# YuyaW-0118/Sparse-Matrix-Linear-Equations

Hardware: AMD Instinct MI355X
Metric: fp64 SpMV GFLOP/s + achieved HBM GB/s vs roofline; CG iters/sec (higher is better)
Workload: dtype f64; 1 GPU; merge-path CSR SpMV fp64, 1 RHS, batch of 4 pwtk-shaped matrices per step per GPU (configs[1]); m=217918, nnz=11524432, batch=4, parallelism=independent SpMV batches, 1 GPU(s)

## Files before the change

include/mspmv.h:

```cpp
#ifndef MSPMV_H
#define MSPMV_H

#include <stddef.h>

#ifndef MSPMV_API
#define MSPMV_API __attribute__((visibility("default")))
#endif

#ifdef __cplusplus
extern "C" {
#endif

typedef enum mspmv_status {
    MSPMV_OK = 0,
    MSPMV_ERR_INVALID = 1,
    MSPMV_ERR_HIP = 2,
    MSPMV_ERR_OOM = 3,
    MSPMV_ERR_BREAKDOWN = 4,
    MSPMV_ERR_RCCL = 5,
    MSPMV_ERR_UNSUPPORTED = 6,
    MSPMV_ERR_IO = 7,
    MSPMV_ERR_STALL = 8,
    MSPMV_ERR_FAULT = 9
} mspmv_status;
// ... 92 lines not shown
MSPMV_API mspmv_status mspmv_color_greedy(const mspmv_csr_d *a, int *colors, int *num_colors);
MSPMV_API mspmv_status mspmv_csr_permute_sym(const mspmv_csr_d *a, const int *perm, int *ro, int *ci, double *va);
MSPMV_API mspmv_status mspmv_ilu0_create_colored(const mspmv_csr_d *a, const int *colors, int device,
                                                 mspmv_ilu0 *out);
MSPMV_API mspmv_status mspmv_ilu0_colors(mspmv_ilu0 m, int *num_colors, int *perm);
MSPMV_API mspmv_status mspmv_ilu0_apply_dev(mspmv_handle a, mspmv_ilu0 m, const double *d_B, double *d_X, int L);
MSPMV_API mspmv_status mspmv_dpbicgstab_ilu0_multi(mspmv_handle a, mspmv_ilu0 m, const double *B, double *X, int L,
                                                   int max_iters, double tolerance, int *iters,
                                                   double *max_err_hist, int hist_cap);
MSPMV_API mspmv_status mspmv_dpbicgstab_ilu0_multi_dev(mspmv_handle a, mspmv_ilu0 m, const double *d_B, double *d_X,
                                                       int L, int max_iters, double tolerance, int *iters,
                                                       double *max_err_hist, int hist_cap);

MSPMV_API mspmv_status mspmv_ic0_create_colored(const mspmv_csr_d *a, const int *colors, int device, double *shift,
                                                mspmv_ic0 *out);
MSPMV_API mspmv_status mspmv_ic0_colors(mspmv_ic0 m, int *num_colors, int *perm);
MSPMV_API mspmv_status mspmv_ic0_apply_dev(mspmv_handle a, mspmv_ic0 m, const double *d_B, double *d_X, int L);

MSPMV_API mspmv_status mspmv_time_spmm_dev(mspmv_handle h, const double *d_X, double *d_Y, int L, int reps,
                                 size_t flush_bytes, double *avg_ms);
MSPMV_API mspmv_status mspmv_time_spmm_batch_dev(int count, const mspmv_handle *hs, const double *const *d_X,
                                                 double *const *d_Y, int L, int reps, double *step_ms,
                                                 double *tile_kernel_ms, int *kernels_per_step);
MSPMV_API mspmv_status mspmv_time_stream_read(int device, size_t bytes, int reps, double *gbps);
MSPMV_API mspmv_status mspmv_last_kernel_ms(mspmv_handle h, double *tile_kernel_ms, int *kernels_per_call);

MSPMV_API mspmv_status mspmv_tile_plan(mspmv_handle h, int L, int *num_tiles, int *tile_items, int *num_carries,
                                       mspmv_coord *bounds);
MSPMV_API mspmv_status mspmv_tile_streams(mspmv_handle h, int *tiles_cols16, int *tiles_dict);
MSPMV_API mspmv_status mspmv_plan_dict_tiles(mspmv_handle h, int L, int *tiles_dict);
MSPMV_API mspmv_status mspmv_plan_block_tiles(mspmv_handle h, int L, int *tiles_blk);
MSPMV_API mspmv_status mspmv_plan_block_rounds(mspmv_handle h, int L, int *tiles_two_rounds);
MSPMV_API mspmv_status mspmv_plan_block_records(mspmv_handle h, int L, int *chunks_compact, int *chunks_escaped);
enum mspmv_slab_stat {
    MSPMV_SLAB_STAT_BLOCKS = 0,
    MSPMV_SLAB_STAT_GROUPS,
    MSPMV_SLAB_STAT_UNITS,
    MSPMV_SLAB_STAT_UNITS_MAX,
    MSPMV_SLAB_STAT_ROWS_MAX,
    MSPMV_SLAB_STAT_EMPTY_BLOCKS,
    MSPMV_SLAB_STAT_CARRIES,
    MSPMV_SLAB_STAT_CHUNKS_FULL,
    MSPMV_SLAB_STAT_CHUNKS_ENTRY_CUT,
    MSPMV_SLAB_STAT_RUNS_CUT,
    MSPMV_SLAB_STAT_CHUNKS_LONG,
    MSPMV_SLAB_STAT_LONG_RUNS_MAX,
    MSPMV_SLAB_STAT_LG0,
    MSPMV_SLAB_STAT_SEGMENTS = MSPMV_SLAB_STAT_LG0 + 7,
    MSPMV_SLAB_STAT_SEGMENTS_MAX,
    MSPMV_SLAB_STAT_SEGMENTS_FULL,
    MSPMV_SLAB_STAT_SEGMENTS_RAGGED,
    MSPMV_SLAB_STAT_PACK_8X1,
    MSPMV_SLAB_STAT_PACK_4X2,
    MSPMV_SLAB_STAT_PACK_2X3,
    MSPMV_SLAB_STAT_PACK_2X4,
    MSPMV_SLAB_STAT_PACK_1X5,
    MSPMV_SLAB_STAT_UNPACKED_1 = MSPMV_SLAB_STAT_PACK_1X5 + 4,
    MSPMV_SLAB_STAT_MEDIUM_2 = MSPMV_SLAB_STAT_UNPACKED_1 + 8,
    MSPMV_SLAB_STAT_SLICES_ODD = MSPMV_SLAB_STAT_MEDIUM_2 + 7,
    MSPMV_SLAB_STAT_SLICES_PARTIAL,
    MSPMV_SLAB_STAT_LONG_1,
    MSPMV_SLAB_STAT_LONG_2,
    MSPMV_SLAB_STAT_LONG_3PLUS,
    MSPMV_SLAB_STAT_PIECES_MAX,
    MSPMV_SLAB_STAT_SEGS_PIECES_ONLY,
    MSPMV_SLAB_STAT_SEGS_REFILL,
// ... 36 lines not shown
```

sparse-matrix-linear-equations_amd/csrc/mspmv_api.hip:

```cpp
#include "mspmv_internal.h"

#include <algorithm>
#include <atomic>
#include <chrono>
#include <cstdio>
#include <cstring>
#include <map>
#include <mutex>
#include <vector>

namespace mspmv {

static thread_local std::string g_err;

void set_error(const std::string &msg) { g_err = msg; }

hipError_t launch_flush(void *p, size_t bytes, hipStream_t s, bool fresh);

}

unsigned long long mspmv_next_generation()
{
    static std::atomic<unsigned long long> next{1};
    return next.fetch_add(1, std::memory_order_relaxed);
// ... 933 lines not shown
    const TilePlan *plan = nullptr;
    ST_TRY(product_plan(h, L, &plan));
    *tiles_blk = plan->d_blk ? plan->num_tiles_blk : 0;
    return MSPMV_OK;
}

mspmv_status mspmv_plan_block_rounds(mspmv_handle h, int L, int *tiles_two_rounds)
{
    ST_TRY(check_handle(h));
    if (!tiles_two_rounds)
        return invalid("null out pointer");
    if (!supported_L(L))
        return (set_error("L must be one of 1, 2, 4, 8, 16"), MSPMV_ERR_UNSUPPORTED);
    const TilePlan *plan = nullptr;
    ST_TRY(product_plan(h, L, &plan));
    *tiles_two_rounds = plan->d_blk ? plan->blk_two_rounds : 0;
    return MSPMV_OK;
}

mspmv_status mspmv_plan_block_records(mspmv_handle h, int L, int *chunks_compact, int *chunks_escaped)
{
    ST_TRY(check_handle(h));
    if (!chunks_compact || !chunks_escaped)
        return invalid("null out pointer");
    if (!supported_L(L))
        return (set_error("L must be one of 1, 2, 4, 8, 16"), MSPMV_ERR_UNSUPPORTED);
    const TilePlan *plan = nullptr;
    ST_TRY(product_plan(h, L, &plan));
    *chunks_compact = plan->d_recs ? plan->blk_rec_compact : 0;
    *chunks_escaped = plan->d_recs ? plan->blk_rec_escaped : 0;
    return MSPMV_OK;
}

mspmv_status mspmv_slab_plan_stats(mspmv_handle h, int L, long long *stats, int count, int *on_slab)
{
    ST_TRY(check_handle(h));
    if (!on_slab || (count > 0 && !stats))
        return invalid("null out pointer");
    if (!supported_L(L))
        return (set_error("L must be one of 1, 2, 4, 8, 16"), MSPMV_ERR_UNSUPPORTED);
    const TilePlan *plan = nullptr;
    ST_TRY(product_plan(h, L, &plan));
    *on_slab = plan->slab ? 1 : 0;
    if (!plan->slab)
        return MSPMV_OK;
    SlabStats s = plan->slab->stats;
    s.v[MSPMV_SLAB_STAT_BLOCKS] = plan->num_tiles;
    s.v[MSPMV_SLAB_STAT_GROUPS] = plan->slab->groups;
    s.v[MSPMV_SLAB_STAT_CARRIES] = plan->num_carries;
    for (int i = 0; i < count && i < MSPMV_SLAB_STAT_COUNT; ++i)
        stats[i] = s.v[i];
    return MSPMV_OK;
}

mspmv_status mspmv_block_record_encode(const unsigned short *offsets, int wc, unsigned *entries, int *escaped)
{
    if (!entries || !escaped || (wc > 0 && !offsets))
        return invalid("null pointer");
    if (wc < 0 || wc > 64)
        return invalid("a chunk holds 0..64 pattern columns");
    *escaped = blk_rec_encode(offsets, wc, entries) ? 0 : 1;
    return MSPMV_OK;
}

mspmv_status mspmv_block_record_decode(const unsigned *record, int q, unsigned *offset)
{
// ... 63 lines not shown
```

sparse-matrix-linear-equations_amd/csrc/mspmv_internal.h:

```cpp
#pragma once

#include <hip/hip_runtime.h>

#include <cstdint>
#include <map>
#include <string>
#include <type_traits>
#include <utility>
#include <vector>

#include "mspmv.h"
#include "mspmv_host.h"

static inline hipError_t memset_sync(void *p, int value, size_t bytes)
{
    const hipError_t e = hipMemset(p, value, bytes);
    return e == hipSuccess ? hipStreamSynchronize(nullptr) : e;
}

namespace mspmv {

constexpr int kBlock = 256;
constexpr unsigned kFaultTicket = 1u;
constexpr int kNnzPad = 16;
// ... 96 lines not shown
    double *d_rem_val = nullptr;
};

struct TilePlan {
    int lanes = kBlock;
    int tile_items = 0;
    int snap = 0;
    int num_tiles = 0;
    int2 *d_bounds = nullptr;
    unsigned char *d_split = nullptr;
    unsigned char *d_modes[5] = {nullptr, nullptr, nullptr, nullptr, nullptr};
    int num_carries = 0;
    double *d_carry_val = nullptr;
    int4 *d_fix = nullptr;
    unsigned *d_fix_cnt = nullptr;
    int carry_L = 0;
    int *d_colbase = nullptr;
    unsigned short *d_cols16 = nullptr;
    int num_tiles16 = 0;
    int *d_dict = nullptr;
    int *d_ndict = nullptr;
    unsigned short *d_idx16 = nullptr;
    int num_tiles_dict = 0;
    uint4 *d_blk = nullptr;
    int blk_stride = 0;
    unsigned short *d_pcols = nullptr;
    unsigned *d_recs = nullptr;
    int blk_rec_compact = 0;
    int blk_rec_escaped = 0;
    int num_tiles_blk = 0;
    int num_tiles_reg = 0;
    int blk_rows_max = 8;
    bool blk_spmv = false;
    int blk_two_rounds = 0;
    std::vector<unsigned char> h_blk_reg;
    SlabData *slab = nullptr;
    DiaData *dia = nullptr;
};

struct CgScalars {
    double rs_old;
    double b_norm;
    double alpha;
    double beta;
    double pAp;
    double rs_new;
    double rs_par[2];
    double omega;
    double rho;
};

struct CgControl {
    int iter;
    int done;
    int iters_out;
    int breakdown;
    int iter_par[2];
    int x_pending;
    unsigned fault;
    unsigned fault_no_stop;
};


struct ResidentCg {
    bool ok = false;
    int G = 0, rpt = 0, nzr = 0;
// ... 463 lines not shown
```

sparse-matrix-linear-equations_amd/csrc/mspmv_kernels.hip:

```cpp
#include "mspmv_internal.h"
#include "mspmv_device.h"

#include <algorithm>
#include <type_traits>
#include <cmath>
#include <cstdio>
#include <cstdlib>

namespace mspmv {


template <typename... KArgs, typename... Args>
static void ggl(void (*kernel)(KArgs...), dim3 grid, dim3 block, hipStream_t s, Args... args)
{
    hipLaunchKernelGGL(kernel, grid, block, 0, s, args...);
}

template <bool NT, typename T>
__device__ __forceinline__ T ld_stream(const T *p)
{
    if (NT)
        return __builtin_nontemporal_load(p);
    return *p;
}
// ... 396 lines not shown
    double *head_pub;
    double *y0;
    int num_tiles;
    CgScalars *scal;
    CgControl *ctrl;
    const unsigned char *conv;
    double *partials;
    unsigned *gtickets;
    double *dot_out;
    int m;
    const double *part_in;
    int n_part_in;
    int parity;
    double tol;
    double *hist;
    int hist_cap;
    const int *colbase;
    const unsigned short *cols16;
    const uint4 *blk;
    int blk_stride;
    int all_reg;
    const unsigned short *pcols;
    const unsigned *recs;
    const int *dict;
    const int *ndict;
    const unsigned short *idx16;
    int ld;
    int early_re;
    int blk_rows_max;
    unsigned long long *stamps;
    int tb;
    int blk_spmv;
    int n;
};

enum : int { kModeSpmv = 0, kModeCg = 1, kModeDot = 2 };

__device__ __forceinline__ double2 cg_rp(const TileArgs &a, long long i)
{
    return reinterpret_cast<const double2 *>(a.x)[i];
}
__device__ __forceinline__ void cg_pstore(const TileArgs &a, long long i, double p) { a.p_new[2 * i + 1] = p; }

__device__ __forceinline__ int pslot(int k) { return k ^ ((k >> 3) & 7); }

template <int TB>
__device__ __forceinline__ void tile_sync()
{
    if (TB == 64) {
        __builtin_amdgcn_fence(__ATOMIC_RELEASE, "wavefront");
        __builtin_amdgcn_wave_barrier();
        __builtin_amdgcn_fence(__ATOMIC_ACQUIRE, "wavefront");
    } else {
        __syncthreads();
    }
}

template <int NJ, bool CG>
struct StageRegs {
    int c[NJ];
    double v[NJ];
    double xv[NJ];
    double pv[CG ? NJ : 1];
};
template <int NJ, bool CG, bool NT, int TB = kBlock>
__device__ __forceinline__ void stage_issue(const TileArgs &a, int n0, int nnzt, int colbase, StageRegs<NJ, CG> &st)
// ... 224 lines not shown
                if (CG)
                    x = x + beta * st.pv[s];
                int start = 0;
#pragma unroll
                for (int i = 0; i < kBlkRows; ++i) {
                    const int len = blk_len(d, i);
                    if (i < h && j < len)
                        s_prod[pslot(vofs + start + j)] = st.v[s][i] * x;
                    start += i < h ? len : 0;
                }
            }
        }
    }
}

__device__ __forceinline__ double rows8_sum(const double (&p)[kBlkRows])
{
    const int lane = threadIdx.x & 63;
    const bool b5 = lane & 32, b4 = lane & 16, b3 = lane & 8;
    double q4[4], q2[2];
#pragma unroll
    for (int k = 0; k < 4; ++k)
        q4[k] = (b5 ? p[k + 4] : p[k]) + __shfl_xor(b5 ? p[k] : p[k + 4], 32);
#pragma unroll
    for (int k = 0; k < 2; ++k)
        q2[k] = (b4 ? q4[k + 2] : q4[k]) + __shfl_xor(b4 ? q4[k] : q4[k + 2], 16);
    double v = (b3 ? q2[1] : q2[0]) + __shfl_xor(b3 ? q2[0] : q2[1], 8);
    v += __shfl_xor(v, 4);
    v += __shfl_xor(v, 2);
    v += __shfl_xor(v, 1);
    return v;
}

__device__ __forceinline__ double rows8_sum32(const double (&p)[kBlkRows])
{
    const int lane = threadIdx.x & 63;
    const bool b4 = lane & 16, b3 = lane & 8, b2 = lane & 4;
    double q4[4], q2[2];
#pragma unroll
    for (int k = 0; k < 4; ++k)
        q4[k] = (b4 ? p[k + 4] : p[k]) + __shfl_xor(b4 ? p[k] : p[k + 4], 16);
#pragma unroll
    for (int k = 0; k < 2; ++k)
        q2[k] = (b3 ? q4[k + 2] : q4[k]) + __shfl_xor(b3 ? q4[k] : q4[k + 2], 8);
    double v = (b2 ? q2[1] : q2[0]) + __shfl_xor(b2 ? q2[0] : q2[1], 4);
    v += __shfl_xor(v, 2);
    v += __shfl_xor(v, 1);
    return v;
}

template <bool NT>
__device__ __forceinline__ unsigned blk_pair_rec(const TileArgs &a, int t, int round)
{
    const int lane = threadIdx.x & 63;
    const int slot = 8 * round + 2 * (int)(threadIdx.x >> 6) + (lane >> 5);
    return ld_stream<NT>(a.recs + ((size_t)t * a.blk_stride + slot) * kRecDwords + (lane & 15));
}

template <bool NT, int KR>
__device__ __forceinline__ void blk_rows_pair(const TileArgs &a, int t, unsigned rec, int nd, int r0, int n0,
                                              int colbase)
{
    constexpr int NW = kBlock / 64;
    const int lane = threadIdx.x & 63;
    const int half = lane >> 5, hl = lane & 31;
    const int wave = __builtin_amdgcn_readfirstlane((int)(threadIdx.x >> 6));
    for (int round = 0; round * 2 * NW < nd; ++round) {
        if (round > 0)
            rec = blk_pair_rec<NT>(a, t, round);
        const int di = wave + NW * (2 * round + half);
        const bool valid = di < nd;
        auto dword = [&](int k) { return (unsigned)__shfl((int)rec, (lane & 32) + k); };
        const uint4 d = make_uint4(dword(0), dword(1), dword(2), dword(3));
        const int vofs = d.x & 0xffff, wc = d.x >> 24;
        const int h = d.y & 15, rofs = d.y >> 16;
        double2 v[KR];
        bool in0[KR], in1[KR];
        int start = 0;
#pragma unroll
        for (int i = 0; i < KR; ++i) {
            const int len = blk_len(d, i);
            in0[i] = valid && i < h && 2 * hl < len;
            in1[i] = valid && i < h && 2 * hl + 1 < len;
            v[i] = make_double2(0.0, 0.0);
            if (in0[i])
                v[i] = ld_stream<NT>(reinterpret_cast<const double2 *>(a.vals + n0 + vofs + start + 2 * hl));
            start += i < h ? len : 0;
        }
        const int q = max(min(2 * hl, wc - 1), 0);
        int e;
        const unsigned E = blk_rec_find([&](int i) { return dword(4 + i); }, q, e);
        const unsigned En = dword(4 + min(e + 1, kRecEntries - 1));
        int c0 = colbase + (int)((E & 0xffffu) + (unsigned)q - (E >> 24));
        int c1 = c0 + 1;
        if (2 * hl + 1 < wc && 2 * hl + 1 == (int)((E >> 24) + ((E >> 16) & 255u)))
            c1 = colbase + (int)(En & 0xffffu);
        if (d.y & kRecEscape) {
            const int p = (d.y >> 4) & 7;
            int pstart = 0;
#pragma unroll
            for (int i = 0; i < KR - 1; ++i)
                pstart += i < p ? blk_len(d, i) : 0;
            unsigned cc = 0u;
            if (2 * hl < wc)
                cc = ld_stream<NT>(reinterpret_cast<const unsigned *>(a.cols16 + n0 + vofs + pstart + 2 * hl));
            c0 = colbase + (int)(cc & 0xffffu);
            c1 = 2 * hl + 1 < wc ? colbase + (int)(cc >> 16) : c0 + 1;
        }
        const int base = min(c0, a.n - 2);
        const double2 xx = *reinterpret_cast<const double2 *>(a.x + base);
        const double x0 = base == c0 ? xx.x : xx.y;
        double x1 = xx.y;
        if (c1 != c0 + 1)
            x1 = a.x[c1];
        double pr[kBlkRows];
#pragma unroll
        for (int i = 0; i < kBlkRows; ++i)
            pr[i] = i < KR ? (in0[i] ? v[i].x * x0 : 0.0) + (in1[i] ? v[i].y * x1 : 0.0) : 0.0;
        const double sum = rows8_sum32(pr);
        const int myrow = hl >> 2;
        if (valid && (hl & 3) == 0 && myrow < h)
            a.y[r0 + rofs + myrow] = sum;
    }
}

template <int MODE, bool NT, int TB, typename Head>
__device__ __forceinline__ void blk_rows(const TileArgs &a, int t, const uint4 &bd, int nd, int r0, int n0,
                                         int colbase, double &beta, double &dot, Head &&head)
{
    constexpr bool CG = MODE == kModeCg;
    constexpr int NW = TB / 64;
    const int lane = threadIdx.x & 63;
    const int wave = __builtin_amdgcn_readfirstlane((int)(threadIdx.x >> 6));
    const int myrow = lane >> 3;
    for (int round = 0; round * 2 * NW < nd; ++round) {
        BlkRegs<CG> st;
        double2 ro[2];
#pragma unroll
        for (int s = 0; s < 2; ++s) {
            const int di = wave + NW * (2 * round + s);
            st.c[s] = 0;
            ro[s] = make_double2(0.0, 0.0);
#pragma unroll
            for (int i = 0; i < kBlkRows; ++i)
                st.v[s][i] = 0.0;
            if (di < nd) {
                const uint4 d = blk_read(bd, di);
                const int vofs = d.x & 0xffff, wc = d.x >> 24;
                const int h = d.y & 15, rofs = d.y >> 16;
                int start = 0;
#pragma unroll
                for (int i = 0; i < kBlkRows; ++i) {
                    const int len = blk_len(d, i);
                    if (i < h && lane < len)
// ... 486 lines not shown
        return;
    const int mean = (nnzt + nseg - 1) / nseg;
    int lg = 0;
    while (lg < 6 && (4 << lg) < mean)
        ++lg;
    const int G = 1 << lg;
    const int lane = threadIdx.x & (G - 1);
    auto col = [&](int k) {
        return colbase >= 0 ? colbase + (int)ld_stream<NT>(a.cols16 + n0 + k) : ld_stream<NT>(a.cols + n0 + k);
    };
    for (int r = (int)threadIdx.x >> lg; r < nseg; r += kBlock >> lg) {
        const int s0 = r == 0 ? 0 : a.row_offsets[r0 + r] - n0;
        const int e = r < nrows ? a.row_offsets[r0 + r + 1] - n0 : nnzt;
        double v = 0.0;
        for (int k = s0 + lane; k < e; k += G)
            v += ld_stream<NT>(a.vals + n0 + k) * a.x[col(k)];
        for (int off = G >> 1; off > 0; off >>= 1)
            v += __shfl_xor(v, off);
        if (lane == 0) {
            if (r < nrows)
                *(r == 0 ? a.y0 : &a.y[r0 + r]) = v;
            else
                store_sc1(&a.carry_val[t], v);
        }
    }
}

struct BlkSmem {
    double red[kBlock / 64];
    double cval[kBlock];
    int last;
};

template <int MODE, bool NT, int KR = kBlkRows, bool FB = false>
__global__ __launch_bounds__(kBlock) void k_spmv_blk(TileArgs a)
{
    constexpr bool CG = MODE == kModeCg;
    __shared__ BlkSmem sm;
    const int tid = threadIdx.x;
    const int stopped = (MODE != kModeSpmv || a.ctrl) ? a.ctrl->done : 0;
    const int t = xcd_tile(blockIdx.x, a.num_tiles);
    const int2 b0 = a.bounds[t];
    const int colbase = a.colbase[t];
    const uint4 bd =
        (tid & 63) < a.blk_stride ? a.blk[(size_t)t * a.blk_stride + (tid & 63)] : make_uint4(0u, 0u, 0u, 0u);
    const int nblk = (int)(((unsigned)__builtin_amdgcn_readfirstlane((int)bd.y) >> 8) & 255u);
    double beta = 0.0, dot = 0.0;
    bool go = true;
    PartRegs<CG ? kUpdateMaxBlocks / kBlock : 1> pin;
    if constexpr (CG)
        part_load(a.part_in, a.n_part_in, pin);
    if constexpr (MODE == kModeSpmv && KR <= 6) {
        const unsigned rec = blk_pair_rec<NT>(a, t, 0);
        asm volatile("" ::"s"(b0.x), "s"(b0.y), "s"(colbase), "v"(rec));
        if (stopped)
            return;
        const int nrec = (int)(((unsigned)__builtin_amdgcn_readlane((int)rec, 1) >> 8) & 255u);
        if constexpr (FB) {
            if (nrec == 0) {
                const int4 fx = load_fix(a, t);
                a.y0 = fx.z > 0 ? a.head_val + t : a.y + b0.x;
                tile_rows_reg<NT>(a, t, b0.x, b0.y, a.cols16 ? colbase : -1);
                close_split_rows<kBlock>(a, t, fx, 1, 1);
                return;
            }
        }
        blk_rows_pair<NT, KR>(a, t, rec, nrec, b0.x, b0.y, colbase);
        return;
    }
    blk_rows<MODE, NT, kBlock>(a, t, bd, nblk, b0.x, b0.y, colbase, beta, dot, [&]() {
        if (stopped)
            go = false;
        else if constexpr (CG)
// ... 786 lines not shown
    return hipGetLastError();
}

static TileArgs make_args(mspmv_handle_s *h, const TilePlan &plan, const double *X, double *Y, int L)
{
    TileArgs a{};
    a.row_offsets = h->d_row_offsets;
    a.m = h->m;
    a.cols = h->d_cols;
    a.vals = h->d_vals;
    a.x = X;
    a.xr = X;
    a.y = Y;
    a.bounds = plan.d_bounds;
    a.split = plan.d_split;
    a.rmode = plan.d_modes[l_index(L)];
    a.carry_val = plan.d_carry_val;
    a.fix = plan.num_carries ? plan.d_fix : nullptr;
    a.fix_cnt = plan.d_fix_cnt;
    a.fault = h->d_fault;
    a.head_val = plan.d_carry_val + (size_t)std::max(plan.num_tiles, 1) * plan.carry_L;
    a.head_pub = a.head_val + (size_t)std::max(plan.num_tiles, 1) * plan.carry_L;
    a.num_tiles = plan.num_tiles;
    if (L == 1 || plan.d_blk) {
        a.colbase = plan.d_colbase;
        a.cols16 = plan.d_cols16;
        a.blk = plan.d_blk;
        a.blk_stride = plan.blk_stride;
        a.pcols = plan.d_pcols;
        a.recs = plan.d_recs;
        a.all_reg = plan.d_blk && plan.num_tiles_reg == plan.num_tiles && (L == 1 || spmm_blk_enabled());
        a.blk_spmv = L == 1 && plan.blk_spmv;
        a.blk_rows_max = plan.blk_rows_max;
    }
    a.dict = plan.d_dict;
    a.ndict = plan.d_ndict;
    a.idx16 = plan.d_idx16;
    a.ld = L;
    a.early_re = L == 1 ? 1 : 0;
    a.tb = L == 1 ? plan.lanes : kBlock;
    a.n = h->n;
    return a;
}

template <int LL, int I, int MODE>
static void launch_spmm_nt(const TileArgs &a, hipStream_t s, bool nt)
{
    if constexpr (MODE != kModeCg) {
        const dim3 grid(a.num_tiles), block(kBlock);
        dispatch_bool(nt, [&](auto ntc) {
            constexpr bool NT = decltype(ntc)::value;
            if constexpr (spmm_dict_max(LL) > 0) {
                if (a.dict) {
                    ggl(k_spmm_tile<LL, I, MODE, NT, true>, grid, block, s, a);
                    return;
                }
            }
            if (MODE == kModeSpmv && !a.fix)
                ggl(k_spmm_tile<LL, I, MODE, NT, false, false>, grid, block, s, a);
            else
                ggl(k_spmm_tile<LL, I, MODE, NT>, grid, block, s, a);
        });
    }
}

template <int LL, int MODE>
static void launch_spmm_L(const TileArgs &a, hipStream_t s, bool nt)
{
    if constexpr (MODE != kModeCg) {
        if (a.all_reg) {
            const dim3 grid(a.num_tiles), block(kBlock);
            dispatch_bool(nt, [&](auto ntc) {
                constexpr bool NT = decltype(ntc)::value;
                if (a.blk_rows_max <= 6)
                    ggl(k_spmm_blk<LL, MODE, NT, 6>, grid, block, s, a);
                else
                    ggl(k_spmm_blk<LL, MODE, NT>, grid, block, s, a);
            });
            return;
        }
    }
    launch_spmm_nt<LL, (LL >= 16 ? 32 : LL >= 8 ? 24 : 8), MODE>(a, s, nt);
}

template <int MODE>
static void launch_spmv_1(const TileArgs &a, hipStream_t s, bool nt)
{
    const dim3 grid(a.num_tiles), block(kBlock);
    dispatch_bool(nt, [&](auto ntc) {
        constexpr bool NT = decltype(ntc)::value;
        if (MODE == kModeSpmv && a.blk_spmv) {
            if (a.all_reg)
                ggl(k_spmv_blk<kModeSpmv, NT, 6>, grid, block, s, a);
            else
                ggl(k_spmv_blk<kModeSpmv, NT, 6, true>, grid, block, s, a);
        } else if (MODE == kModeDot && a.all_reg) {
            ggl(k_spmv_blk<kModeDot, NT>, grid, block, s, a);
        } else if (MODE == kModeSpmv && a.tb == 64) {
            ggl(k_spmv_tile<kSpmvIpt, kModeSpmv, NT, 64>, grid, dim3(64), s, a);
        } else if (MODE == kModeCg && !a.blk) {
            ggl(k_spmv_tile<kSpmvIpt, MODE, NT, kBlock, false>, grid, block, s, a);
        } else if (MODE == kModeSpmv && !a.fix) {
            ggl(k_spmv_tile<kSpmvIpt, MODE, NT, kBlock, true, false>, grid, block, s, a);
        } else {
            ggl(k_spmv_tile<kSpmvIpt, MODE, NT>, grid, block, s, a);
        }
    });
}

template <int MODE>
static hipError_t launch_tile(const TileArgs &a, int L, hipStream_t s, bool nt)
{
    if (MODE == kModeCg && L != 1)
        return hipErrorInvalidValue;
    return dispatch_L(L, [&](auto Lc) {
        constexpr int LL = decltype(Lc)::value;
        if constexpr (LL == 1)
            launch_spmv_1<MODE>(a, s, nt);
        else
            launch_spmm_L<LL, MODE>(a, s, nt);
        return hipGetLastError();
    });
}

hipError_t launch_spmv_tile_stamped(mspmv_handle_s *h, const TilePlan &plan, const double *d_x, double *d_y,
                                   unsigned long long *d_stamps)
{
    TileArgs a = make_args(h, plan, d_x, d_y, 1);
    if (a.blk_spmv || a.tb == 64 || plan.dia || plan.slab)
        return hipErrorNotSupported;
    a.stamps = d_stamps;
    const dim3 grid(a.num_tiles), block(kBlock);
    if (plan.num_tiles == 0)
        return hipSuccess;
    const bool nt = stream_nt(h);
    dispatch_bool(nt, [&](auto ntc) {
        constexpr bool NT = decltype(ntc)::value;
        if (!a.fix)
            ggl(k_spmv_tile<kSpmvIpt, kModeSpmv, NT, kBlock, true, false, true>, grid, block, h->stream, a);
        else
            ggl(k_spmv_tile<kSpmvIpt, kModeSpmv, NT, kBlock, true, true, true>, grid, block, h->stream, a);
    });
    return hipGetLastError();
}

hipError_t launch_spmm_tile_only(mspmv_handle_s *h, const TilePlan &plan, const double *d_X, double *d_Y, int L,
                                 int ld, CgControl *ctrl)
{
    if (plan.num_tiles == 0)
        return hipSuccess;
    if (plan.dia)
        return launch_dia(h, plan, d_X, d_Y, L, ld, ctrl);
    if (plan.slab) {
        if (plan.slab->L != L || (L == 1 && ctrl))
            return hipErrorInvalidValue;
        return L == 1 ? launch_slab(h, plan, d_X, d_Y) : launch_slab_mm(h, plan, d_X, d_Y, L, ld, ctrl);
// ... 89 lines not shown
```

sparse-matrix-linear-equations_amd/csrc/mspmv_plan.hip:

```cpp
#include "mspmv_internal.h"

#include <algorithm>
#include <cstdlib>
#include <vector>

using namespace mspmv;

void mspmv::free_plan(TilePlan &p)
{
    dev_free(p.d_bounds);
    dev_free(p.d_split);
    for (auto &m : p.d_modes)
        dev_free(m);
    dev_free(p.d_fix);
    dev_free(p.d_fix_cnt);
    dev_free(p.d_carry_val);
    dev_free(p.d_colbase);
    dev_free(p.d_cols16);
    dev_free(p.d_dict);
    dev_free(p.d_ndict);
    dev_free(p.d_idx16);
    dev_free(p.d_blk);
    dev_free(p.d_pcols);
    dev_free(p.d_recs);
// ... 2 lines not shown
    free_dia(p.dia);
    p.dia = nullptr;
}

static mspmv_status build_plan(mspmv_handle_s *h, int L, const TilePlan **out, int lanes = 0,
                               const std::vector<int2> *fixed = nullptr);

static mspmv_status ensure_modes(mspmv_handle_s *h, TilePlan &p, int L)
{
    unsigned char *&m = p.d_modes[l_index(L)];
    if (m)
        return MSPMV_OK;
    mspmv_status st = dev_alloc(&m, (size_t)std::max(p.num_tiles, 1));
    if (st != MSPMV_OK)
        return st;
    hipError_t e = launch_tile_modes(h->d_row_offsets, p.d_bounds, p.d_split, p.num_tiles, L, m, h->stream, p.lanes);
    if (e == hipSuccess)
        e = hipStreamSynchronize(h->stream);
    if (e != hipSuccess) {
        set_error(std::string("tile modes: ") + hipGetErrorString(e));
        dev_free(m);
        m = nullptr;
        return MSPMV_ERR_HIP;
    }
    return MSPMV_OK;
}

static int env_tristate(const char *name)
{
    const char *e = getenv(name);
    return e && *e ? (atoi(e) != 0 ? 1 : 0) : -1;
}

static mspmv_status optional_failed(mspmv_status st, bool forced)
{
    if (forced && st != MSPMV_ERR_UNSUPPORTED)
        return st;
    set_error("");
    (void)hipGetLastError();
    return MSPMV_OK;
}

static mspmv_status keep_optional(mspmv_handle_s *h, int key, TilePlan &p, mspmv_status st, bool forced, int *decision)
{
    if (st != MSPMV_OK) {
        free_plan(p);
        return optional_failed(st, forced);
    }
    h->plans.emplace(key, p);
    *decision = 1;
    return MSPMV_OK;
}

constexpr double kDiaAutoFill = 0.85;
constexpr double kDiaWindowFill = 0.3;

static mspmv_status dia_decide(mspmv_handle_s *h)
{
    h->dia = 0;
    const int sw = env_tristate("MSPMV_DIA");
    if (sw == 0)
        return MSPMV_OK;
    TilePlan p;
    const mspmv_status st = build_dia_plan(h, p, sw == 1 ? 0.0 : kDiaAutoFill, sw == 1 ? 0.0 : kDiaWindowFill);
    return keep_optional(h, kDiaPlanKey, p, st, sw == 1, &h->dia);
}
// ... 189 lines not shown
    if (single && !onewave && p.d_cols16 && spmv_blocks_enabled()) {
        if ((st = dev_alloc(&p.d_blk, (size_t)T * kBlkPerTile)) != MSPMV_OK)
            return fail(st);
        e = launch_build_blocks(h->d_row_offsets, h->d_cols, p.d_bounds, p.d_split, p.d_colbase, T, p.d_blk,
                                h->stream, kBlkPlanChunks);
        std::vector<uint4> hd((size_t)T * kBlkPerTile);
        if (e == hipSuccess)
            e = hipMemcpyAsync(hd.data(), p.d_blk, sizeof(uint4) * hd.size(), hipMemcpyDeviceToHost, h->stream);
        if (e == hipSuccess)
            e = hipStreamSynchronize(h->stream);
        if (e != hipSuccess) {
            set_error(std::string("node blocks: ") + hipGetErrorString(e));
            return fail(MSPMV_ERR_HIP);
        }
        p.h_blk_reg.assign((size_t)T, 0);
        int maxnd = 0, maxh = 0;
        std::vector<unsigned char> reg((size_t)T, 0);
        for (int t = 0; t < T; ++t) {
            const uint4 *d = &hd[(size_t)t * kBlkPerTile];
            const int nd = (int)((d[0].y >> 8) & 255u);
            if (nd == 0)
                continue;
            ++p.num_tiles_blk;
            maxnd = std::max(maxnd, nd);
            for (int i = 0; i < nd; ++i)
                maxh = std::max(maxh, (int)(d[i].y & 15u));
            bool one = true;
            for (int i = 0; i < nd; ++i)
                one = one && ((d[i].x >> 16) & 255u) == 0;
            reg[(size_t)t] = one;
            p.num_tiles_reg += one;
        }
        p.blk_spmv = p.num_tiles_reg > 0 && 2LL * p.num_tiles_reg >= T;
        for (int t = 0; t < T; ++t) {
            const int nd = (int)((hd[(size_t)t * kBlkPerTile].y >> 8) & 255u);
            p.h_blk_reg[(size_t)t] = p.blk_spmv || (reg[(size_t)t] && nd <= kBlkTileChunks);
            p.blk_two_rounds += nd > kBlkTileChunks;
        }
        dev_free(p.d_blk);
        p.d_blk = nullptr;
        p.blk_rows_max = maxh > 0 ? maxh : 8;
        if (p.num_tiles_blk > 0) {
            p.blk_stride = maxnd <= 8 ? 8 : maxnd <= 16 ? 16 : maxnd <= 32 ? 32 : 64;
            std::vector<uint4> packed((size_t)T * p.blk_stride, make_uint4(0u, 0u, 0u, 0u));
            for (int t = 0; t < T; ++t)
                for (int i = 0, nd = (int)((hd[(size_t)t * kBlkPerTile].y >> 8) & 255u); i < nd; ++i)
                    packed[(size_t)t * p.blk_stride + i] = hd[(size_t)t * kBlkPerTile + i];
            if ((st = dev_alloc(&p.d_blk, packed.size())) != MSPMV_OK)
                return fail(st);
            if (hipMemcpy(p.d_blk, packed.data(), sizeof(uint4) * packed.size(), hipMemcpyHostToDevice) != hipSuccess) {
                set_error("node blocks: upload failed");
                return fail(MSPMV_ERR_HIP);
            }
            const size_t np = packed.size() * 64;
            if ((st = dev_alloc(&p.d_pcols, np)) != MSPMV_OK)
                return fail(st);
            e = hipMemsetAsync(p.d_pcols, 0, sizeof(unsigned short) * np, h->stream);
            if (e == hipSuccess)
                e = launch_fill_pcols(p.d_blk, p.blk_stride, p.d_bounds, p.d_cols16, T, p.d_pcols, h->stream);
            if (e == hipSuccess)
                e = hipStreamSynchronize(h->stream);
            if (e != hipSuccess) {
                set_error(std::string("node blocks: pattern-column slots: ") + hipGetErrorString(e));
                return fail(MSPMV_ERR_HIP);
            }
            int *d_counts = nullptr;
// ... 304 lines not shown
```

sparse-matrix-linear-equations_amd/mspmv/__init__.py:

```python
from __future__ import annotations

import atexit
import ctypes
import itertools
import os
import weakref
from dataclasses import dataclass
from typing import Optional

import numpy as np

_HERE = os.path.dirname(os.path.abspath(__file__))
LIB_PATH = os.environ.get("MSPMV_LIB") or os.path.join(_HERE, "libmspmv.so")

SIMPLE, MERGE, NONZERO_SPLIT = 0, 1, 2

STATUS = {
    0: "OK", 1: "INVALID", 2: "HIP", 3: "OOM", 4: "BREAKDOWN", 5: "RCCL", 6: "UNSUPPORTED", 7: "IO",
    8: "STALL", 9: "FAULT",
}
FAULT = 9
POISON_FILL, POISON_LATE_ZERO, POISON_NO_STOP = 1, 2, 4
SUPPORTED_L = (1, 2, 4, 8, 16)

# ... 74 lines not shown
    "mspmv_ic0_create": (_I, [ctypes.POINTER(_CsrD), _I, ctypes.POINTER(_P)]),
    "mspmv_csr_transpose": (_I, [ctypes.POINTER(_CsrD), _P, _P, _P]),
    "mspmv_ic0_destroy": (_I, [_P]),
    "mspmv_dpcg_ic0_multi": (_I, [_P, _P, _P, _P, _I, _I, _D, _I, _PI, _P, _I]),
    "mspmv_dpcg_ic0_multi_dev": (_I, [_P, _P, _P, _P, _I, _I, _D, _I, _PI, _P, _I]),
    "mspmv_ic0_solve_dev": (_I, [_P, _P, _I, _P, _P, _I]),
    "mspmv_ic0_create_colored": (_I, [ctypes.POINTER(_CsrD), _P, _I, _PD, ctypes.POINTER(_P)]),
    "mspmv_ic0_colors": (_I, [_P, _PI, _P]),
    "mspmv_ic0_apply_dev": (_I, [_P, _P, _P, _P, _I]),
    "mspmv_ilu0_values": (_I, [ctypes.POINTER(_CsrD), _P]),
    "mspmv_ilu0_create": (_I, [ctypes.POINTER(_CsrD), _I, ctypes.POINTER(_P)]),
    "mspmv_ilu0_destroy": (_I, [_P]),
    "mspmv_ilu0_solve_dev": (_I, [_P, _P, _I, _P, _P, _I]),
    "mspmv_color_greedy": (_I, [ctypes.POINTER(_CsrD), _P, _PI]),
    "mspmv_csr_permute_sym": (_I, [ctypes.POINTER(_CsrD), _P, _P, _P, _P]),
    "mspmv_ilu0_create_colored": (_I, [ctypes.POINTER(_CsrD), _P, _I, ctypes.POINTER(_P)]),
    "mspmv_ilu0_colors": (_I, [_P, _PI, _P]),
    "mspmv_ilu0_apply_dev": (_I, [_P, _P, _P, _P, _I]),
    "mspmv_dpbicgstab_ilu0_multi": (_I, [_P, _P, _P, _P, _I, _I, _D, _PI, _P, _I]),
    "mspmv_dpbicgstab_ilu0_multi_dev": (_I, [_P, _P, _P, _P, _I, _I, _D, _PI, _P, _I]),
    "mspmv_dpcg_spai_multi": (_I, [_P, _P, _P, _P, _I, _I, _D, _I, _PI, _P, _I]),
    "mspmv_dpcg_spai_multi_dev": (_I, [_P, _P, _P, _P, _I, _I, _D, _I, _PI, _P, _I]),
    "mspmv_time_spmm_dev": (_I, [_P, _P, _P, _I, _I, _SZ, _PD]),
    "mspmv_time_stream_read": (_I, [_I, _SZ, _I, _PD]),
    "mspmv_last_kernel_ms": (_I, [_P, _PD, _PI]),
    "mspmv_time_spmm_batch_dev": (_I, [_I, ctypes.POINTER(_P), ctypes.POINTER(_P), ctypes.POINTER(_P), _I, _I,
                                       _PD, _PD, _PI]),
    "mspmv_tile_plan": (_I, [_P, _I, _PI, _PI, _PI, ctypes.POINTER(Coord)]),
    "mspmv_tile_streams": (_I, [_P, _PI, _PI]),
    "mspmv_plan_dict_tiles": (_I, [_P, _I, _PI]),
    "mspmv_plan_block_tiles": (_I, [_P, _I, _PI]),
    "mspmv_plan_block_rounds": (_I, [_P, _I, _PI]),
    "mspmv_plan_block_records": (_I, [_P, _I, _PI, _PI]),
    "mspmv_slab_plan_stats": (_I, [_P, _I, _P, _I, _PI]),
    "mspmv_block_record_encode": (_I, [_P, _I, _P, _PI]),
    "mspmv_block_record_decode": (_I, [_P, _I, ctypes.POINTER(ctypes.c_uint)]),
    "mspmv_tile_modes": (_I, [_P, _I, _P]),
    "mspmv_tile_lanes": (_I, [_P, _I, _PI]),
    "mspmv_offset_windows": (_I, [ctypes.POINTER(_CsrD), _D, _D, _PI, _PI, ctypes.POINTER(ctypes.c_longlong), _PI, _P,
                                  ctypes.POINTER(ctypes.c_longlong)]),
    "mspmv_spmv_kernel_name": (ctypes.c_char_p, [_P]),
    "mspmv_spmm_kernel_name": (ctypes.c_char_p, [_P, _I]),
    "mspmv_cg_kernel_name": (ctypes.c_char_p, [_P]),
    "mspmv_solver_product_kernel_name": (ctypes.c_char_p, [_P]),
    "mspmv_device_malloc": (_I, [_I, _SZ, ctypes.POINTER(_P)]),
    "mspmv_device_free": (_I, [_P]),
    "mspmv_memcpy_h2d": (_I, [_P, _P, _SZ]),
    "mspmv_memcpy_d2h": (_I, [_P, _P, _SZ]),
    "mspmv_memcpy_d2d": (_I, [_P, _P, _SZ]),
    "mspmv_memset_dev": (_I, [_P, _I, _SZ]),
    "mspmv_synth_banded": (_I, [_I, ctypes.c_longlong, _I, ctypes.c_ulonglong, _P, _P, _P]),
    "mspmv_market_read": (_I, [ctypes.c_char_p, _D, _PI, _PI, _PI, ctypes.POINTER(_P), ctypes.POINTER(_P),
                               ctypes.POINTER(_P)]),
    "mspmv_generate": (_I, [_I, _I, _I, _D, _PI, _PI, _PI, ctypes.POINTER(_P), ctypes.POINTER(_P), ctypes.POINTER(_P)]),
    "mspmv_host_free": (None, [_P]),
    "mspmv_dist_partition": (_I, [_P, _I, _I, _I, _P]),
    "mspmv_dist_localize": (_I, [_P, _I, _I, _P, _P, _P, _PI, _P, _I, _P]),
    "mspmv_comm_unique_id": (_I, [_P]),
    "mspmv_dist_create": (_I, [_P, _I, _I, _I, _P, ctypes.POINTER(_CsrD), ctypes.POINTER(_P)]),
    "mspmv_comm_create": (_I, [_P, _I, _I, _I, ctypes.POINTER(_P)]),
    "mspmv_comm_destroy": (_I, [_P]),
    "mspmv_dist_create_on": (_I, [_P, _P, ctypes.POINTER(_CsrD), ctypes.POINTER(_P)]),
    "mspmv_dist_destroy": (_I, [_P]),
    "mspmv_dist_info": (_I, [_P, _PI, _PI, _PI]),
    "mspmv_dist_spmm_dev": (_I, [_P, _P, _P, _I]),
    "mspmv_dist_x_ext": (_I, [_P, _I, ctypes.POINTER(_P)]),
# ... 340 lines not shown

    def cg_kernel_name(self) -> str:
        return lib.mspmv_cg_kernel_name(self.h).decode()

    def solver_product_kernel_name(self) -> str:
        return lib.mspmv_solver_product_kernel_name(self.h).decode()

    def cg_resident_stamps(self, db: "DeviceBuffer", dx: "DeviceBuffer", max_iters: int, tolerance: float,
                           stamp_iters: int):
        it, G = ctypes.c_int(), ctypes.c_int()
        st = np.zeros(stamp_iters * 1024 * 5, np.uint64)
        _check(lib.mspmv_cg_resident_stamps(self.h, db.ptr, dx.ptr, max_iters, tolerance, ctypes.byref(it),
                                            _ptr(st), stamp_iters, ctypes.byref(G)), "cg_resident_stamps")
        return it.value, st[: stamp_iters * G.value * 5].reshape(stamp_iters, G.value, 5)

    def spmm_kernel_name(self, L: int) -> str:
        return lib.mspmv_spmm_kernel_name(self.h, L).decode()

    def plan_block_tiles(self, L: int = 1) -> int:
        n = ctypes.c_int()
        _check(lib.mspmv_plan_block_tiles(self.h, L, ctypes.byref(n)), "plan_block_tiles")
        return n.value

    def plan_block_rounds(self, L: int = 1) -> int:
        n = ctypes.c_int()
        _check(lib.mspmv_plan_block_rounds(self.h, L, ctypes.byref(n)), "plan_block_rounds")
        return n.value

    def plan_block_records(self, L: int = 1):
        c, e = ctypes.c_int(), ctypes.c_int()
        _check(lib.mspmv_plan_block_records(self.h, L, ctypes.byref(c), ctypes.byref(e)), "plan_block_records")
        return c.value, e.value

    def slab_plan_stats(self, L: int = 1):
        out = np.zeros(len(SLAB_STATS), np.int64)
        on = ctypes.c_int()
        _check(lib.mspmv_slab_plan_stats(self.h, L, _ptr(out), out.size, ctypes.byref(on)), "slab_plan_stats")
        return dict(zip(SLAB_STATS, (int(v) for v in out))) if on.value else None

    def spmv(self, x: np.ndarray) -> np.ndarray:
        x = np.ascontiguousarray(x, np.float64)
        assert x.shape == (self.num_cols,)
        y = np.empty(self.num_rows, np.float64)
        _check(lib.mspmv_dspmv(self.h, _ptr(x), _ptr(y)), "dspmv")
        return y

    def spmm(self, X: np.ndarray) -> np.ndarray:
        X = np.ascontiguousarray(X, np.float64)
        L = X.shape[1]
        assert X.shape == (self.num_cols, L)
        Y = np.empty((self.num_rows, L), np.float64)
        _check(lib.mspmv_dspmm(self.h, _ptr(X), _ptr(Y), L), "dspmm")
        return Y

    def spmm_dev(self, dX: DeviceBuffer, dY: DeviceBuffer, L: int = 1, sync: bool = True):
        _check(lib.mspmv_dspmm_dev(self.h, dX.ptr, dY.ptr, L), "dspmm_dev")
        if sync:
            self.sync()

    def time_spmm(self, dX: DeviceBuffer, dY: DeviceBuffer, L: int, reps: int, flush_bytes: int = 0):
        ms = ctypes.c_double()
        _check(lib.mspmv_time_spmm_dev(self.h, dX.ptr, dY.ptr, L, reps, flush_bytes, ctypes.byref(ms)), "time")
        kms, kpc = ctypes.c_double(), ctypes.c_int()
        _check(lib.mspmv_last_kernel_ms(self.h, ctypes.byref(kms), ctypes.byref(kpc)), "last_kernel_ms")
        return ms.value, kms.value, kpc.value

# ... 600 lines not shown
```

Measured before the change: 1333 GFLOP/s.

## Add persistent block-walker path for register-only block SpMV with lower register pressure

Routes the all-register KR=6 block SpMV through a new walker routine that strides over tiles per XCD and prefetches the next tile's bounds, column base and record. It reloads kernel arguments from the kernarg segment, uses ds_bpermute shuffles with a recomputed lane id, and requests 8 waves per EU, all aimed at cutting scalar and vector register use to raise occupancy. The walker grid size is controlled by an environment variable. By default the grid still equals the tile count, so each workgroup handles one tile and the prefetch mostly goes unused. The occupancy hint risks register spills, and the commit also adds optional timestamp instrumentation and an API that reports the walker count.

New measurement: 1298 GFLOP/s. -2.6%, worse.

```diff
diff --git a/include/mspmv.h b/include/mspmv.h
--- a/include/mspmv.h
+++ b/include/mspmv.h
@@ -148,6 +148,7 @@
 MSPMV_API mspmv_status mspmv_plan_block_tiles(mspmv_handle h, int L, int *tiles_blk);
 MSPMV_API mspmv_status mspmv_plan_block_rounds(mspmv_handle h, int L, int *tiles_two_rounds);
 MSPMV_API mspmv_status mspmv_plan_block_records(mspmv_handle h, int L, int *chunks_compact, int *chunks_escaped);
+MSPMV_API mspmv_status mspmv_plan_block_walkers(mspmv_handle h, int *workgroups);
 enum mspmv_slab_stat {
     MSPMV_SLAB_STAT_BLOCKS = 0,
     MSPMV_SLAB_STAT_GROUPS,
diff --git a/sparse-matrix-linear-equations_amd/csrc/mspmv_api.hip b/sparse-matrix-linear-equations_amd/csrc/mspmv_api.hip
--- a/sparse-matrix-linear-equations_amd/csrc/mspmv_api.hip
+++ b/sparse-matrix-linear-equations_amd/csrc/mspmv_api.hip
@@ -989,6 +989,17 @@
     return MSPMV_OK;
 }
 
+mspmv_status mspmv_plan_block_walkers(mspmv_handle h, int *workgroups)
+{
+    ST_TRY(check_handle(h));
+    if (!workgroups)
+        return invalid("null out pointer");
+    const TilePlan *plan = nullptr;
+    ST_TRY(product_plan(h, 1, &plan));
+    *workgroups = !plan->blk_spmv || plan->slab || plan->dia ? 0 : plan->blk_walkers > 0 ? plan->blk_walkers : plan->num_tiles;
+    return MSPMV_OK;
+}
+
 mspmv_status mspmv_slab_plan_stats(mspmv_handle h, int L, long long *stats, int count, int *on_slab)
 {
     ST_TRY(check_handle(h));
diff --git a/sparse-matrix-linear-equations_amd/csrc/mspmv_internal.h b/sparse-matrix-linear-equations_amd/csrc/mspmv_internal.h
--- a/sparse-matrix-linear-equations_amd/csrc/mspmv_internal.h
+++ b/sparse-matrix-linear-equations_amd/csrc/mspmv_internal.h
@@ -152,6 +152,7 @@
     int num_tiles_reg = 0;
     int blk_rows_max = 8;
     bool blk_spmv = false;
+    int blk_walkers = 0;
     int blk_two_rounds = 0;
     std::vector<unsigned char> h_blk_reg;
     SlabData *slab = nullptr;
diff --git a/sparse-matrix-linear-equations_amd/csrc/mspmv_kernels.hip b/sparse-matrix-linear-equations_amd/csrc/mspmv_kernels.hip
--- a/sparse-matrix-linear-equations_amd/csrc/mspmv_kernels.hip
+++ b/sparse-matrix-linear-equations_amd/csrc/mspmv_kernels.hip
@@ -452,6 +452,7 @@
     int tb;
     int blk_spmv;
     int n;
+    int blk_walkers;
 };
 
 enum : int { kModeSpmv = 0, kModeCg = 1, kModeDot = 2 };
@@ -742,45 +743,110 @@
     return v;
 }
 
-__device__ __forceinline__ double rows8_sum32(const double (&p)[kBlkRows])
-{
-    const int lane = threadIdx.x & 63;
+__device__ __forceinline__ int lane_now()
+{
+    int l;
+    asm volatile("v_mbcnt_lo_u32_b32 %0, -1, 0\n\tv_mbcnt_hi_u32_b32 %0, -1, %0" : "=v"(l));
+    return l;
+}
+template <bool OWN>
+__device__ __forceinline__ int shfl_lane(int v, int src)
+{
+    if constexpr (OWN)
+        return __builtin_amdgcn_ds_bpermute(src << 2, v);
+    else
+        return __shfl(v, src);
+}
+template <bool OWN>
+__device__ __forceinline__ double shfl_xor_lane(double v, int mask, int lane)
+{
+    if constexpr (OWN) {
+        const int src = (lane ^ mask) << 2;
+        const int lo = __builtin_amdgcn_ds_bpermute(src, __double2loint(v));
+        const int hi = __builtin_amdgcn_ds_bpermute(src, __double2hiint(v));
+        return __hiloint2double(hi, lo);
+    } else {
+        return __shfl_xor(v, mask);
+    }
+}
+template <bool OWN = false>
+__device__ __forceinline__ double rows8_sum32(const double (&p)[kBlkRows], unsigned tid = threadIdx.x)
+{
+    const int lane = tid & 63;
     const bool b4 = lane & 16, b3 = lane & 8, b2 = lane & 4;
     double q4[4], q2[2];
 #pragma unroll
     for (int k = 0; k < 4; ++k)
-        q4[k] = (b4 ? p[k + 4] : p[k]) + __shfl_xor(b4 ? p[k] : p[k + 4], 16);
+        q4[k] = (b4 ? p[k + 4] : p[k]) + shfl_xor_lane<OWN>(b4 ? p[k] : p[k + 4], 16, lane);
 #pragma unroll
     for (int k = 0; k < 2; ++k)
-        q2[k] = (b3 ? q4[k + 2] : q4[k]) + __shfl_xor(b3 ? q4[k] : q4[k + 2], 8);
-    double v = (b2 ? q2[1] : q2[0]) + __shfl_xor(b2 ? q2[0] : q2[1], 4);
-    v += __shfl_xor(v, 2);
-    v += __shfl_xor(v, 1);
+        q2[k] = (b3 ? q4[k + 2] : q4[k]) + shfl_xor_lane<OWN>(b3 ? q4[k] : q4[k + 2], 8, lane);
+    double v = (b2 ? q2[1] : q2[0]) + shfl_xor_lane<OWN>(b2 ? q2[0] : q2[1], 4, lane);
+    v += shfl_xor_lane<OWN>(v, 2, lane);
+    v += shfl_xor_lane<OWN>(v, 1, lane);
     return v;
 }
 
 template <bool NT>
-__device__ __forceinline__ unsigned blk_pair_rec(const TileArgs &a, int t, int round)
-{
-    const int lane = threadIdx.x & 63;
-    const int slot = 8 * round + 2 * (int)(threadIdx.x >> 6) + (lane >> 5);
+__device__ __forceinline__ unsigned blk_pair_rec(const TileArgs &a, int t, int round, unsigned tid = threadIdx.x)
+{
+    const int lane = tid & 63;
+    const int slot = 8 * round + 2 * (int)(tid >> 6) + (lane >> 5);
     return ld_stream<NT>(a.recs + ((size_t)t * a.blk_stride + slot) * kRecDwords + (lane & 15));
 }
 
-template <bool NT, int KR>
+struct BlkLab {
+    unsigned long long t0;
+    unsigned d[3];
+};
+#ifdef MSPMV_BLK_LAB_STAMPS
+constexpr int kBlkLabTiles = 8192, kBlkLabWaves = kBlock / 64;
+__device__ unsigned long long g_blk_lab_stamps[(size_t)kBlkLabTiles * kBlkLabWaves * 4];
+#define BLK_LAB_ENTRY(lab) (lab).t0 = __builtin_amdgcn_s_memtime()
+#define BLK_LAB_MARK(lab, i) (lab).d[i] = (unsigned)(__builtin_amdgcn_s_memtime() - (lab).t0)
+#define BLK_LAB_LANDED(lab)                                                                       \
+    do {                                                                                          \
+        if (lab) {                                                                                \
+            asm volatile("s_waitcnt vmcnt(0)" ::: "memory");                                      \
+            BLK_LAB_MARK(*(lab), 1);                                                              \
+        }                                                                                         \
+    } while (0)
+__device__ __forceinline__ void blk_lab_store(const BlkLab &lab, int t, unsigned tid)
+{
+    if (t < kBlkLabTiles && (tid & 63) == 0) {
+        unsigned long long *o = g_blk_lab_stamps + ((size_t)t * kBlkLabWaves + (tid >> 6)) * 4;
+        o[0] = lab.t0;
+        o[1] = lab.d[0];
+        o[2] = lab.d[1];
+        o[3] = lab.d[2];
+    }
+}
+#else
+#define BLK_LAB_ENTRY(lab) ((void)0)
+#define BLK_LAB_MARK(lab, i) ((void)0)
+#define BLK_LAB_LANDED(lab) ((void)0)
+#endif
+
+template <bool NT, int KR, typename Later = std::nullptr_t>
 __device__ __forceinline__ void blk_rows_pair(const TileArgs &a, int t, unsigned rec, int nd, int r0, int n0,
-                                              int colbase)
+                                              int colbase, unsigned tid = threadIdx.x, BlkLab *lab = nullptr,
+                                              Later &&later = nullptr)
 {
     constexpr int NW = kBlock / 64;
-    const int lane = threadIdx.x & 63;
-    const int half = lane >> 5, hl = lane & 31;
-    const int wave = __builtin_amdgcn_readfirstlane((int)(threadIdx.x >> 6));
-    for (int round = 0; round * 2 * NW < nd; ++round) {
-        if (round > 0)
-            rec = blk_pair_rec<NT>(a, t, round);
+    constexpr bool OWN = !std::is_same_v<std::decay_t<Later>, std::nullptr_t>;
+    const int wave = __builtin_amdgcn_readfirstlane((int)(tid >> 6));
+    for (int round = 0; (OWN && round == 0) || round * 2 * NW < nd; ++round) {
+        const int lane = OWN ? lane_now() : (int)(tid & 63);
+        const int half = lane >> 5, hl = lane & 31;
+        if (round > 0) {
+            if constexpr (!OWN)
+                rec = blk_pair_rec<NT>(a, t, round, tid);
+            else
+                rec = later(round, lane);
+        }
         const int di = wave + NW * (2 * round + half);
         const bool valid = di < nd;
-        auto dword = [&](int k) { return (unsigned)__shfl((int)rec, (lane & 32) + k); };
+        auto dword = [&](int k) { return (unsigned)shfl_lane<OWN>((int)rec, (lane & 32) + k); };
         const uint4 d = make_uint4(dword(0), dword(1), dword(2), dword(3));
         const int vofs = d.x & 0xffff, wc = d.x >> 24;
         const int h = d.y & 15, rofs = d.y >> 16;
@@ -823,13 +889,15 @@
         double x1 = xx.y;
         if (c1 != c0 + 1)
             x1 = a.x[c1];
+        BLK_LAB_LANDED(lab);
         double pr[kBlkRows];
 #pragma unroll
         for (int i = 0; i < kBlkRows; ++i)
             pr[i] = i < KR ? (in0[i] ? v[i].x * x0 : 0.0) + (in1[i] ? v[i].y * x1 : 0.0) : 0.0;
-        const double sum = rows8_sum32(pr);
-        const int myrow = hl >> 2;
-        if (valid && (hl & 3) == 0 && myrow < h)
+        const int fl = OWN ? lane_now() : lane, fhl = fl & 31;
+        const double sum = rows8_sum32<OWN>(pr, fl);
+        const int myrow = fhl >> 2;
+        if (valid && (fhl & 3) == 0 && myrow < h)
             a.y[r0 + rofs + myrow] = sum;
     }
 }
@@ -1382,13 +1450,93 @@
     int last;
 };
 
+typedef const __attribute__((address_space(4))) char *KernArg;
+__device__ __forceinline__ KernArg kernarg_again()
+{
+    KernArg kp = (KernArg)__builtin_amdgcn_kernarg_segment_ptr();
+    asm volatile("" : "+s"(kp));
+    return kp;
+}
+
+template <bool NT, int KR>
+__device__ __forceinline__ void blk_walk(const TileArgs &a, const int2 *__restrict__ bounds,
+                                         const int *__restrict__ colbases, const unsigned *__restrict__ recs,
+                                         int stopped)
+{
+    const int T = a.num_tiles, xk = blockIdx.x & 7;
+    const int cnt = (T >> 3) + (xk < (T & 7)), base = xk * (T >> 3) + min(xk, T & 7);
+    const int S = (int)((gridDim.x + 7) >> 3);
+    int i = blockIdx.x >> 3;
+    if (i >= cnt)
+        return;
+    [[maybe_unused]] BlkLab lab;
+    BLK_LAB_ENTRY(lab);
+    auto record = [&](int t, unsigned tid) {
+        const unsigned ofs = (2u * (tid >> 6) + ((tid >> 5) & 1u)) * kRecDwords + (tid & 15u);
+        return ld_stream<NT>(recs + (size_t)t * a.blk_stride * kRecDwords + ofs);
+    };
+    int t = base + i;
+    int2 b0 = bounds[t];
+    int colbase = colbases[t];
+    const unsigned ws = 64u * (unsigned)__builtin_amdgcn_readfirstlane((int)(threadIdx.x >> 6));
+    unsigned rec = record(t, threadIdx.x);
+    asm volatile("" ::"s"(b0.x), "s"(b0.y), "s"(colbase), "v"(rec));
+    if (stopped)
+        return;
+    for (;;) {
+        i += S;
+        const bool more = i < cnt;
+        const int tn = more ? base + i : t;
+        const int2 b1 = bounds[tn];
+        const int cb1 = colbases[tn];
+        const unsigned rec1 = record(tn, ws + (unsigned)lane_now());
+        const int nrec = (int)(((unsigned)__builtin_amdgcn_readlane((int)rec, 1) >> 8) & 255u);
+        BLK_LAB_MARK(lab, 0);
+        const KernArg kp = kernarg_again();
+        TileArgs la = a;
+        la.x = *(const double *const __attribute__((address_space(4))) *)(kp + offsetof(TileArgs, x));
+        la.y = *(double *const __attribute__((address_space(4))) *)(kp + offsetof(TileArgs, y));
+        la.cols16 = *(const unsigned short *const __attribute__((address_space(4))) *)(kp + offsetof(TileArgs, cols16));
+        la.n = *(const __attribute__((address_space(4))) int *)(kp + offsetof(TileArgs, n));
+        auto later = [&](int round, int lane) {
+            const KernArg kq = kernarg_again();
+            const unsigned *rq = *(const unsigned *const __attribute__((address_space(4))) *)(kq + offsetof(TileArgs, recs));
+            const int stride = *(const __attribute__((address_space(4))) int *)(kq + offsetof(TileArgs, blk_stride));
+            unsigned w = ws;
+            asm volatile("" : "+s"(w));
+            const unsigned ofs = (8u * round + (w >> 5) + ((unsigned)lane >> 5)) * kRecDwords + ((unsigned)lane & 15u);
+            return ld_stream<NT>(rq + (size_t)t * stride * kRecDwords + ofs);
+        };
+#ifdef MSPMV_BLK_LAB_STAMPS
+        blk_rows_pair<NT, KR>(la, t, rec, nrec, b0.x, b0.y, colbase, ws, &lab, later);
+        BLK_LAB_MARK(lab, 2);
+        blk_lab_store(lab, t, ws + (unsigned)lane_now());
+#else
+        blk_rows_pair<NT, KR>(la, t, rec, nrec, b0.x, b0.y, colbase, ws, nullptr, later);
+#endif
+        if (!more)
+            return;
+        asm volatile("" ::"v"(rec1));
+        BLK_LAB_ENTRY(lab);
+        t = tn;
+        b0 = b1;
+        colbase = cb1;
+        rec = rec1;
+    }
+}
+
 template <int MODE, bool NT, int KR = kBlkRows, bool FB = false>
-__global__ __launch_bounds__(kBlock) void k_spmv_blk(TileArgs a)
+__global__ __launch_bounds__(kBlock)
+__attribute__((amdgpu_waves_per_eu(MODE == kModeSpmv && KR <= 6 && !FB ? 8 : 1, 8))) void k_spmv_blk(TileArgs a)
 {
     constexpr bool CG = MODE == kModeCg;
     __shared__ BlkSmem sm;
     const int tid = threadIdx.x;
     const int stopped = (MODE != kModeSpmv || a.ctrl) ? a.ctrl->done : 0;
+    if constexpr (MODE == kModeSpmv && KR <= 6 && !FB) {
+        blk_walk<NT, KR>(a, a.bounds, a.colbase, a.recs, stopped);
+        return;
+    }
     const int t = xcd_tile(blockIdx.x, a.num_tiles);
     const int2 b0 = a.bounds[t];
     const int colbase = a.colbase[t];
@@ -2241,6 +2389,7 @@
         a.all_reg = plan.d_blk && plan.num_tiles_reg == plan.num_tiles && (L == 1 || spmm_blk_enabled());
         a.blk_spmv = L == 1 && plan.blk_spmv;
         a.blk_rows_max = plan.blk_rows_max;
+        a.blk_walkers = L == 1 ? plan.blk_walkers : 0;
     }
     a.dict = plan.d_dict;
     a.ndict = plan.d_ndict;
@@ -2300,7 +2449,7 @@
         constexpr bool NT = decltype(ntc)::value;
         if (MODE == kModeSpmv && a.blk_spmv) {
             if (a.all_reg)
-                ggl(k_spmv_blk<kModeSpmv, NT, 6>, grid, block, s, a);
+                ggl(k_spmv_blk<kModeSpmv, NT, 6>, dim3(a.blk_walkers > 0 ? a.blk_walkers : a.num_tiles), block, s, a);
             else
                 ggl(k_spmv_blk<kModeSpmv, NT, 6, true>, grid, block, s, a);
         } else if (MODE == kModeDot && a.all_reg) {
@@ -2331,6 +2480,23 @@
         return hipGetLastError();
     });
 }
+
+#ifdef MSPMV_BLK_LAB_STAMPS
+}
+extern "C" __attribute__((visibility("default"))) int mspmv_lab_blk_stamps(unsigned long long *host, int n)
+{
+    using namespace mspmv;
+    const int all = kBlkLabTiles * kBlkLabWaves * 4;
+    const int m = std::min(n, all);
+    if (hipMemcpyFromSymbol(host, HIP_SYMBOL(g_blk_lab_stamps), sizeof(unsigned long long) * (size_t)m) != hipSuccess)
+        return -1;
+    static const std::vector<unsigned long long> zero((size_t)all, 0ull);
+    if (hipMemcpyToSymbol(HIP_SYMBOL(g_blk_lab_stamps), zero.data(), sizeof(unsigned long long) * (size_t)all) != hipSuccess)
+        return -1;
+    return m;
+}
+namespace mspmv {
+#endif
 
 hipError_t launch_spmv_tile_stamped(mspmv_handle_s *h, const TilePlan &plan, const double *d_x, double *d_y,
                                    unsigned long long *d_stamps)
diff --git a/sparse-matrix-linear-equations_amd/csrc/mspmv_plan.hip b/sparse-matrix-linear-equations_amd/csrc/mspmv_plan.hip
--- a/sparse-matrix-linear-equations_amd/csrc/mspmv_plan.hip
+++ b/sparse-matrix-linear-equations_amd/csrc/mspmv_plan.hip
@@ -58,6 +58,21 @@
     return e && *e ? (atoi(e) != 0 ? 1 : 0) : -1;
 }
 
+constexpr int kBlkWalkSgprs = 78;
+static int blk_walk_grid(const mspmv_handle_s *h, int T)
+{
+    const char *e = getenv("MSPMV_BLK_WALKERS");
+    const long long n = e && *e ? atoll(e) : -1;
+    if (n == 0 || T <= 0)
+        return T;
+    if (n > 0)
+        return (int)std::min<long long>((n + 7) / 8 * 8, 1 << 30);
+    const int per_cu = std::min(8, 800 / ((kBlkWalkSgprs + 15) / 16 * 16 + 16));
+    const long long resident = std::max(8LL, (long long)h->num_cus * per_cu / 8 * 8);
+    (void)resident;
+    return T;
+}
+
 static mspmv_status optional_failed(mspmv_status st, bool forced)
 {
     if (forced && st != MSPMV_ERR_UNSUPPORTED)
@@ -313,6 +328,7 @@
             p.num_tiles_reg += one;
         }
         p.blk_spmv = p.num_tiles_reg > 0 && 2LL * p.num_tiles_reg >= T;
+        p.blk_walkers = p.blk_spmv && p.num_tiles_reg == T ? blk_walk_grid(h, T) : T;
         for (int t = 0; t < T; ++t) {
             const int nd = (int)((hd[(size_t)t * kBlkPerTile].y >> 8) & 255u);
             p.h_blk_reg[(size_t)t] = p.blk_spmv || (reg[(size_t)t] && nd <= kBlkTileChunks);
diff --git a/sparse-matrix-linear-equations_amd/mspmv/__init__.py b/sparse-matrix-linear-equations_amd/mspmv/__init__.py
--- a/sparse-matrix-linear-equations_amd/mspmv/__init__.py
+++ b/sparse-matrix-linear-equations_amd/mspmv/__init__.py
@@ -130,6 +130,7 @@
     "mspmv_plan_block_tiles": (_I, [_P, _I, _PI]),
     "mspmv_plan_block_rounds": (_I, [_P, _I, _PI]),
     "mspmv_plan_block_records": (_I, [_P, _I, _PI, _PI]),
+    "mspmv_plan_block_walkers": (_I, [_P, _PI]),
     "mspmv_slab_plan_stats": (_I, [_P, _I, _P, _I, _PI]),
     "mspmv_block_record_encode": (_I, [_P, _I, _P, _PI]),
     "mspmv_block_record_decode": (_I, [_P, _I, ctypes.POINTER(ctypes.c_uint)]),
@@ -536,6 +537,11 @@
         _check(lib.mspmv_plan_block_records(self.h, L, ctypes.byref(c), ctypes.byref(e)), "plan_block_records")
         return c.value, e.value
 
+    def plan_block_walkers(self) -> int:
+        n = ctypes.c_int()
+        _check(lib.mspmv_plan_block_walkers(self.h, ctypes.byref(n)), "plan_block_walkers")
+        return n.value
+
     def slab_plan_stats(self, L: int = 1):
         out = np.zeros(len(SLAB_STATS), np.int64)
         on = ctypes.c_int()
```
